# elucideye/acf

Hardware: AMD Instinct MI355X
Metric: detector FPS @1080p, 8 scales/octave, FACE80 model (higher is better)
Workload: dtype f32

## Files before the change

### acf_amd/csrc/kernels_levels.hip.h

```cpp
#pragma once

namespace acfhip
{

struct RsX
{
    int xa, m;
    float w[4];
    int wofs;
    bool border;
};

__device__ __forceinline__ float rs_C(int xmode, int ha, const RsX& X, const float* __restrict__ ft,
    const float* __restrict__ A, int row)
{
    if (row >= ha)
    {
        return 0.f;
    }
    const float* A0 = A + int64_t(X.xa) * ha + row;
    if (xmode == RS_EXACT)
    {
        float s = A0[0] + A0[ha];
        if (X.m > 2)
// ... 240 lines not shown
        const float a5 = Ac0[r4], b5 = Ac1[r4];
        float ar[5], br[5];
#pragma unroll
        for (int i = 0; i < 5; i++)
        {
            const int j = sh + i;
            ar[i] = j == 0 ? a4.x : (j == 1 ? a4.y : (j == 2 ? a4.z : (j == 3 ? a4.w : a5)));
            br[i] = j == 0 ? b4.x : (j == 1 ? b4.y : (j == 2 ? b4.z : (j == 3 ? b4.w : b5)));
        }
        float C[5];
#pragma unroll
        for (int i = 0; i < 5; i++)
        {
            const float c = border ? ar[i] : ar[i] * w0 + br[i] * w1;
            C[i] = live[i] ? c : 0.f;
        }
        float v[4];
#pragma unroll
        for (int k = 0; k < 4; k++)
        {
            const float c0 = i0[k] == 0 ? C[0] : (i0[k] == 1 ? C[1] : (i0[k] == 2 ? C[2] : C[3]));
            const float c1 = i0[k] == 0 ? C[1] : (i0[k] == 1 ? C[2] : (i0[k] == 2 ? C[3] : C[4]));
            const float o1 = c0 * wy0[k];
            v[k] = one[k] ? o1 : o1 + c1 * wy1[k];
        }
        if (act)
        {
            *reinterpret_cast<float4*>(B + int64_t(xb) * hb + yb0) = make_float4(v[0], v[1], v[2], v[3]);
        }
    }
}

struct RankFn
{
    int32_t shift, base, nbm1;
    uint32_t mask;
};
__device__ __forceinline__ uint4 rank_fetch(float v, const RankFn& f, const uint4* rec, uint32_t& low)
{
    const int key = __float_as_int(v);
    int b;
    asm("v_med3_i32 %0, %1, 0, %2" : "=v"(b) : "v"((key >> f.shift) - f.base), "v"(f.nbm1));
    low = (uint32_t(key) & f.mask) | 0x8000u;
    return rec[b];
}
__device__ __forceinline__ uint32_t rank_count(float v, const uint4& r, uint32_t low)
{
    static_assert(RANK_WINDOW == 7 && sizeof(RankRec) == 16 && RANK_UNUSED == 0x8000, "record layout");
    const uint32_t X = low | (low << 16);
    const uint32_t m0 = (X - r.x) & 0x00008000u;
    const uint32_t m1 = (X - r.y) & 0x80008000u;
    const uint32_t m2 = (X - r.z) & 0x80008000u;
    const uint32_t m3 = (X - r.w) & 0x80008000u;
    const uint32_t n = uint32_t(__builtin_popcount(m0 | (m1 >> 1) | (m2 >> 2) | (m3 >> 3))) + (r.x >> 16);
    return v < 0.f ? 0u : n;
}
__device__ __forceinline__ uint32_t rank_cell(float v, const RankFn& f, const uint4* rec)
{
    uint32_t low;
    const uint4 r = rank_fetch(v, f, rec, low);
    return rank_count(v, r, low);
}

__device__ __forceinline__ RankFn rank_tables_to_lds(const RankChan& rc, const RankRec* __restrict__ recG, uint4* recL, int tid, int nThreads)
{
    const uint4* src = reinterpret_cast<const uint4*>(recG + rc.recOff);
    for (int i = tid; i < rc.nb; i += nThreads)
    {
        recL[i] = src[i];
    }
    RankFn f;
    f.shift = rc.shift;
    f.base = rc.base;
    f.nbm1 = rc.nb - 1;
    f.mask = (1u << rc.shift) - 1u;
    return f;
}

struct RankJob
{
    int64_t src_off;
    int64_t dst_off;
    int32_t hP, wP, pitchR, pad_;
};
constexpr int RANK_CHUNK_COLS = 64;
__global__ void __launch_bounds__(256) k_rank(const float* __restrict__ pyr, int64_t pyr_fs, uint16_t* __restrict__ out, int64_t out_fs,
    const RankJob* __restrict__ jobs, int nChns, const RankChan* __restrict__ chan, const RankRec* __restrict__ recG)
{
    extern __shared__ uint4 ldsRec[];
    const int lvl = blockIdx.y / nChns, z = blockIdx.y - lvl * nChns;
    const RankJob J = jobs[lvl];
    const int c0 = blockIdx.x * RANK_CHUNK_COLS;
    if (c0 >= J.wP)
    {
        return;
    }
    const RankFn fn = rank_tables_to_lds(chan[z], recG, ldsRec, threadIdx.x, 256);
    __syncthreads();
    const float* __restrict__ src = pyr + int64_t(blockIdx.z) * pyr_fs + J.src_off + int64_t(z) * J.hP * J.wP;
    uint16_t* __restrict__ dst = out + int64_t(blockIdx.z) * out_fs + J.dst_off + int64_t(z) * J.pitchR * J.wP;
    const int c1 = min(c0 + RANK_CHUNK_COLS, J.wP);
    const int lane = threadIdx.x & 63, wv = threadIdx.x >> 6;
    for (int c = c0 + wv; c < c1; c += 4)
    {
        for (int r = lane; r < J.hP; r += 64)
        {
            dst[int64_t(c) * J.pitchR + r] = uint16_t(rank_cell(src[int64_t(c) * J.hP + r], fn, ldsRec));
        }
    }
}

struct LevelJob
{
    int32_t hC, wC, out_cs, desc;
    int32_t kind, pad_;
    int64_t in_off;
    int64_t raw_off;
    int64_t out_off;
    int64_t in_ps, out_ps;
    int64_t rank_off, rank_ps;
    int32_t rank_cs, pad2_;
};


typedef uint32_t u32x8 __attribute__((ext_vector_type(8)));
typedef const __attribute__((address_space(4))) u32x8* cptr8_t;

enum
{
    LM_REAL = 0,
    LM_DD = 1,
    LM_DU = 2,
    LM_UD = 3,
    LM_UU = 4
};

typedef __amdgpu_buffer_rsrc_t srd_t;
__device__ __forceinline__ srd_t make_srd(const void* base, int64_t bytes)
{
    const uint64_t a = reinterpret_cast<uint64_t>(base);
    const uint32_t lo = __builtin_amdgcn_readfirstlane(uint32_t(a)), hi = __builtin_amdgcn_readfirstlane(uint32_t(a >> 32));
    const uint32_t n = __builtin_amdgcn_readfirstlane(uint32_t(bytes > 0xffffffffll ? 0xffffffffll : bytes));
    void* p = reinterpret_cast<void*>((uint64_t(hi) << 32) | lo);
    return __builtin_amdgcn_make_buffer_rsrc(p, 0, int(n), 0x00020000);
}
__device__ __forceinline__ float buf_ld(srd_t r, uint32_t voff, uint32_t soff)
{
    return __uint_as_float(__builtin_amdgcn_raw_buffer_load_b32(r, voff, soff, 0));
}
__device__ __forceinline__ void buf_st(srd_t r, uint32_t voff, uint32_t soff, float v)
{
    __builtin_amdgcn_raw_buffer_store_b32(__float_as_uint(v), r, voff, soff, 0);
}

#ifndef ACF_LEVEL_WAVES
#define ACF_LEVEL_WAVES 4
#endif
constexpr int LEVEL_WAVES = ACF_LEVEL_WAVES;
constexpr int LEVEL_RING_FLOATS = 2304;
constexpr int LEVEL_RING_FLOATS_RANK = 1920;

template <int R, int MODE, int RING = LEVEL_RING_FLOATS>
struct LevelWindow
{
    static constexpr bool XDOWN = MODE == LM_DD || MODE == LM_DU;
    static constexpr bool YDOWN = MODE == LM_DD || MODE == LM_UD;
    static constexpr int NY = YDOWN ? 3 : 2;
    static constexpr int JX = XDOWN ? 3 : 2;
    static constexpr int RS = YDOWN ? (3 * R + 1) / 2 : R;
    static constexpr int NBRAW = RING / (RS * 64);
    static constexpr int NB = NBRAW > 12 ? 12 : (NBRAW < JX + 2 ? JX + 2 : NBRAW);
    static constexpr int LA = NB - JX;
    static constexpr int LDS_FLOATS = RS * 64 * (NB + 1);
    static_assert(LA * RS <= 63, "vmcnt immediate");

    uint32_t srow[RS];
    int issued;
    float* ring;

    __device__ __forceinline__ void request(srd_t A, int col, int ha, int wa) const
    {
        const uint32_t cb = uint32_t(min(col, wa - 1)) * uint32_t(ha) * 4u;
        float* slot = ring + (uint32_t(col) % uint32_t(NB)) * (RS * 64);
#pragma unroll
        for (int r = 0; r < RS; r++)
        {
            __builtin_amdgcn_raw_ptr_buffer_load_lds(A, (lptr_t)(slot + 64 * r), 4, srow[r], cb, 0, 0);
        }
    }

    __device__ __forceinline__ void init(srd_t A, float* ring_, int lane, int ha, int wa, int xa0)
    {
#pragma unroll
        for (int r = 0; r < RS; r++)
        {
            srow[r] = lane + 64 * r < ha ? 4u * uint32_t(lane + 64 * r) : 0x40000000u;
        }
        ring = ring_;
        for (int k = 0; k < JX + LA; k++)
        {
            request(A, xa0 + k, ha, wa);
        }
        issued = xa0 + JX + LA - 1;
    }

    __device__ __forceinline__ void advance(srd_t A, int xa, int ha, int wa)
    {
        const int target = xa + JX - 1 + LA;
        while (issued < target)
        {
            issued++;
            request(A, issued, ha, wa);
        }
    }

    __device__ __forceinline__ void read(float (&d)[JX][RS], int xa, int lane) const
    {
        asm volatile("s_waitcnt vmcnt(%0)" ::"n"(LA * RS) : "memory");
#pragma unroll
        for (int j = 0; j < JX; j++)
        {
            const float* slot = ring + (uint32_t(xa + j) % uint32_t(NB)) * (RS * 64) + lane;
#pragma unroll
            for (int r = 0; r < RS; r++)
            {
                d[j][r] = slot[64 * r];
            }
        }
    }
};

template <int R>
struct LaneTaps
{
    uint32_t roff[R][3];
    float wy[R][3];
    uint32_t one[R];
};

template <int R, int MODE, int RING>
__device__ __forceinline__ void level_column(float (&v)[R], int xb, srd_t A, int h, const uint32_t (&yoff)[R],
    int ha, int wa, int ny, const u32x8& xr, const LaneTaps<R>& tp, srd_t raw, bool haveRaw, bool lastOk,
    LevelWindow<R, MODE == LM_REAL ? LM_DD : MODE, RING>& win, float* ldsCol, int lane)
{
    if (MODE == LM_REAL)
    {
        const uint32_t col = uint32_t(xb) * uint32_t(h) * 4u;
#pragma unroll
        for (int k = 0; k < R; k++)
        {
            v[k] = buf_ld(A, yoff[k], col);
        }
        return;
    }
    constexpr bool XDOWN = MODE == LM_DD || MODE == LM_DU;
    constexpr bool YDOWN = MODE == LM_DD || MODE == LM_UD;
    typedef LevelWindow<R, MODE == LM_REAL ? LM_DD : MODE, RING> Win;
    constexpr int NY = Win::NY;
    constexpr int JX = Win::JX;
    const int xa = int(xr[0]), m = int(xr[1]);
    const bool border = xr[3] != 0;
    float w[4] = { __uint_as_float(xr[4]), __uint_as_float(xr[5]), __uint_as_float(xr[6]), __uint_as_float(xr[7]) };
    constexpr int RS = Win::RS;
    if (RS >= 3 && RS < 6)
    {
        ACF_PIN_V(w[0]);
        ACF_PIN_V(w[1]);
        ACF_PIN_V(w[2]);
    }
    win.advance(A, xa, ha, wa);
    float sc[JX][RS];
    win.read(sc, xa, lane);
    float Cr[RS];
    if (XDOWN)
    {
        if (m == 2)
        {
#pragma unroll
            for (int r = 0; r < RS; r++)
            {
                Cr[r] = sc[0][r] * w[0] + sc[1][r] * w[1];
            }
        }
        else if (m >= 3)
        {
#pragma unroll
            for (int r = 0; r < RS; r++)
            {
                Cr[r] = sc[0][r] * w[0] + sc[1][r] * w[1] + sc[JX - 1][r] * w[2];
            }
        }
        else
        {
#pragma unroll
            for (int r = 0; r < RS; r++)
            {
                Cr[r] = sc[0][r] * w[0];
            }
        }
    }
    else if (border)
    {
#pragma unroll
        for (int r = 0; r < RS; r++)
        {
            Cr[r] = sc[0][r];
        }
    }
    else
    {
#pragma unroll
        for (int r = 0; r < RS; r++)
        {
            Cr[r] = sc[0][r] * w[0] + sc[1][r] * w[1];
        }
    }
#pragma unroll
    for (int r = 0; r < RS; r++)
    {
        ldsCol[lane + 64 * r] = Cr[r];
    }
    float C[R][NY];
#pragma unroll
    for (int k = 0; k < R; k++)
    {
#pragma unroll
        for (int o = 0; o < NY; o++)
        {
            C[k][o] = *reinterpret_cast<const float*>(reinterpret_cast<const char*>(ldsCol) + tp.roff[k][o]);
        }
    }
    if (YDOWN)
    {
        if (ny > 2)
        {
#pragma unroll
            for (int k = 0; k < R; k++)
            {
                v[k] = C[k][0] * tp.wy[k][0] + C[k][1] * tp.wy[k][1] + C[k][2] * tp.wy[k][2];
            }
        }
        else
        {
#pragma unroll
            for (int k = 0; k < R; k++)
            {
                v[k] = C[k][0] * tp.wy[k][0] + C[k][1] * tp.wy[k][1];
            }
        }
    }
    else
    {
#pragma unroll
        for (int k = 0; k < R; k++)
        {
            const float o1 = C[k][0] * tp.wy[k][0];
            const float o2 = o1 + C[k][1] * tp.wy[k][1];
            v[k] = tp.one[k] ? o1 : o2;
        }
    }
    if (haveRaw)
    {
        const uint32_t rc = uint32_t(xb) * uint32_t(h) * 4u;
#pragma unroll
        for (int k = 0; k < R; k++)
        {
            if (k < R - 1 || lastOk)
            {
                buf_st(raw, yoff[k], rc, v[k]);
            }
        }
    }
}

enum
{
    LO_F32 = 1,
    LO_RANK = 2
};
struct LevelRank
{
    uint16_t* out;
    int64_t fs;
    RankFn fn;
    const uint4* rec;
};

struct LevelSeg
{
    int x0, x1, xs;
    float* spec;
    float* tru;
};

template <int R, int MODE, int OUT, int SEG>
__device__ __forceinline__ void level_body(const LevelJob& J, const int64_t f, const float* __restrict__ chns, float* __restrict__ pyr, float* __restrict__ rawOut,
    const ResampleDesc* __restrict__ descs, const int32_t* __restrict__ it, const float* __restrict__ ft,
    int nChns, int64_t chns_fs, int64_t pyr_fs, float p, float* __restrict__ dump, float* ldsBlock, int ldsWaveFloats, const LevelRank& rk,
    const LevelSeg& sg)
{
    const int z = __builtin_amdgcn_readfirstlane(blockIdx.x);
    const int lane = threadIdx.x & 63;
    const int h = J.hC, w = J.wC;
    const srd_t Osrd = make_srd(pyr + f * pyr_fs + J.out_off + int64_t(z) * J.out_ps, (int64_t(w - 1) * J.out_cs + h) * 4);
    const int par = int(J.rank_off & 1);
    const srd_t Rsrd = (OUT & LO_RANK) ? make_srd(rk.out + f * rk.fs + (J.rank_off - par) + int64_t(z) * J.rank_ps, (int64_t(w - 1) * J.rank_cs + h + 1 + par) * 2) : Osrd;
    srd_t A, raw = Osrd;
    bool haveRaw = false;
    int ha = 0, wa = 0, ny = 0;
    LaneTaps<R> tp;
    uint32_t yoff[R];
#pragma unroll
    for (int k = 0; k < R; k++)
    {
        yoff[k] = 4u * uint32_t(min(lane + 64 * k, h - 1));
    }
    const bool lastOk = lane + 64 * (R - 1) < h;
    const int32_t* xcol = it;
    if (MODE == LM_REAL)
    {
        A = make_srd(chns + f * chns_fs + J.in_off + int64_t(z) * J.in_ps, J.in_ps * 4);
    }
    else
    {
        const ResampleDesc& d = descs[J.desc];
        A = make_srd(chns + f * chns_fs + d.src_off + int64_t(z) * d.ha * d.wa, int64_t(d.ha) * d.wa * 4);
        haveRaw = rawOut != nullptr;
        if (haveRaw)
        {
            raw = make_srd(rawOut + f * chns_fs + J.raw_off + int64_t(z) * J.in_ps, J.in_ps * 4);
        }
        const int ty = z < d.c1 ? 0 : (z < d.c2 ? 1 : 2);
        const float r = d.r[ty];
        const int hb = d.hb;
        ha = d.ha;
        wa = d.wa;
        xcol = it + d.x_col;
        constexpr bool YDOWN = MODE == LM_DD || MODE == LM_UD;
        typedef LevelWindow<R, MODE == LM_REAL ? LM_DD : MODE> Win0;
        ny = YDOWN ? d.ybd0 : 2;
#pragma unroll
        for (int k = 0; k < R; k++)
        {
            const int ybc = int(yoff[k] >> 2);
            int ya;
            tp.wy[k][0] = tp.wy[k][1] = tp.wy[k][2] = 0.f;
            tp.one[k] = 0;
            if (YDOWN)
            {
                const int q0 = it[d.y_start + ybc];
                ya = it[d.y_src + q0];
#pragma unroll
                for (int o = 0; o < 3; o++)
                {
                    if (o < d.ybd0)
                    {
                        tp.wy[k][o] = ft[d.y_wt + q0 + o] * r;
                    }
                }
            }
            else
            {
                ya = it[d.y_src + ybc];
                tp.wy[k][0] = ft[d.y_wt + ybc] * r;
                tp.wy[k][1] = r - tp.wy[k][0];
                tp.one[k] = (ybc < d.ybd0 || ybc >= hb - d.ybd1) ? 1u : 0u;
            }
#pragma unroll
            for (int o = 0; o < 3; o++)
            {
                tp.roff[k][o] = 4u * uint32_t(min(ya + o, 64 * Win0::RS - 1));
            }
        }
    }
    float nrm = 1.0f / ((p + 2) * (p + 2));
    const float p1 = 1 + p;
    float pv = p;
    if (R <= 5)
    {
        ACF_PIN_V(nrm);
        ACF_PIN_V(pv);
    }
    cptr8_t xrec = (cptr8_t)(uintptr_t)xcol;
    const u32x8 zrec = { 0, 0, 0, 0, 0, 0, 0, 0 };
    float b0[R], b1[R], b2[R], b3[R], prev[R];
#pragma unroll
    for (int k = 0; k < R; k++)
    {
        b0[k] = b1[k] = b2[k] = b3[k] = prev[k] = 0.f;
    }
    const int xs = SEG ? sg.xs : 0, x0 = SEG ? sg.x0 : 0, x1 = SEG ? sg.x1 : w;
    u32x8 xr = (MODE == LM_REAL) ? zrec : xrec[xs];
    u32x8 xrn = (MODE == LM_REAL) ? zrec : xrec[min(xs + 1, w - 1)];
    constexpr int RING = (OUT & LO_RANK) ? LEVEL_RING_FLOATS_RANK : LEVEL_RING_FLOATS;
    typedef LevelWindow<R, MODE == LM_REAL ? LM_DD : MODE, RING> Win;
    Win lw;
    float* ldsCol = ldsBlock + (threadIdx.x >> 6) * ldsWaveFloats;
    if (MODE != LM_REAL)
    {
        lw.init(A, ldsCol + Win::RS * 64, lane, ha, wa, int(xr[0]));
    }
    const int lastLane = (h - 1) & 63;
#define LV_LOAD(FAR, COL)                                                                                           \
    {                                                                                                               \
        level_column<R, MODE, RING>(FAR, min((COL), w - 1), A, h, yoff, ha, wa, ny, xr, tp, raw, haveRaw, lastOk, lw, ldsCol, lane); \
        xr = xrn;                                                                                                   \
        xrn = (MODE == LM_REAL) ? zrec : xrec[min((COL) + 2, w - 1)];                                               \
    }
#define LV_FILTER(I, CUR, NXT)                                                                                      \
    {                                                                                                               \
        const int i_ = (I);                                                                                         \
        float T[R], up[R], dn[R];                                                                                   \
        _Pragma("unroll") for (int k = 0; k < R; k++)                                                               \
        {                                                                                                           \
            const float Im = CUR[k];                                                                                \
            const float Ir = (i_ < w - 1) ? NXT[k] : Im;                                                            \
            const float Il = (i_ == xs) ? Im : prev[k];  \
            T[k] = nrm * (Il + pv * Im + Ir);                                                                       \
            up[k] = wave_ror1(T[k]);                                                    \
            dn[k] = wave_rol1(T[k]);                                                    \
        }                                                                                                           \
        _Pragma("unroll") for (int k = 0; k < R; k++)                                                               \
        {                                                                                                           \
            const int y = lane + 64 * k;                                                                            \
            const float tm = (lane == 0) ? up[k > 0 ? k - 1 : 0] : up[k];                              \
            const float tpv = (lane == 63) ? dn[k + 1 < R ? k + 1 : k] : dn[k];                        \
            const float mid = tm + pv * T[k] + tpv;                                                                 \
             \
             \
            float o = mid;                                                                                          \
            if (k == R - 1)                                                                                         \
            {                                                                                                       \
                o = (y == h - 1) ? tm + p1 * T[k] : o;                                                              \
            }                                                                                                       \
            if (k == 0)                                                                                             \
            {                                                                                                       \
                o = (y == 0) ? p1 * T[k] + tpv : o;                                                                 \
            }                                                                                                       \
            prev[k] = o;                                                                                            \
             \
             \
            const float ov = (k < R - 1 || lastOk) ? o : __int_as_float(__builtin_amdgcn_readlane(__float_as_int(o), lastLane)); \
            if (OUT & LO_F32)                                                                                       \
            {                                                                                                       \
                   \
                buf_st(Osrd, yoff[k], (!SEG || i_ >= x0) ? uint32_t(i_) * uint32_t(J.out_cs) * 4u : 0x40000000u, ov); \
            }                                                                                                       \
        }                                                                                                           \
    }
    uint4 rrec[R];
    uint32_t rlow[R];
    uint32_t rvoff[R];
    if (OUT & LO_RANK)
    {
#pragma unroll
        for (int k = 0; k < R; k++)
        {
            const int y = lane + 64 * k;
            rvoff[k] = (((y + par) & 1) && y <= h) ? uint32_t(2 * (y - 1 + par)) : 0x40000000u;
        }
    }
#define LV_RANK_FETCH()                                                                                             \
    if (OUT & LO_RANK)                                                                                              \
    {                                                                                                               \
        _Pragma("unroll") for (int k = 0; k < R; k++)                                                               \
        {                                                                                                           \
            rrec[k] = rank_fetch(prev[k], rk.fn, rk.rec, rlow[k]);                                                  \
        }                                                                                                           \
    }
#define LV_RANK_STORE(COL)                                                                                          \
    if (OUT & LO_RANK)                                                                                              \
    {                                                                                                               \
        const int c_ = (COL);                                                                                       \
        const uint32_t so_ = c_ >= x0 ? uint32_t(c_) * uint32_t(J.rank_cs) * 2u : 0x40000000u;                      \
        uint32_t n_[R], up_[R];                                                                                     \
        _Pragma("unroll") for (int k = 0; k < R; k++)                                                               \
        {                                                                                                           \
            n_[k] = rank_count(prev[k], rrec[k], rlow[k]);                                                          \
            up_[k] = __float_as_uint(wave_ror1(__uint_as_float(n_[k])));        \
        }                                                                                                           \
        _Pragma("unroll") for (int k = 0; k < R; k++)                                                               \
        {                                                                                                           \
            const uint32_t lo_ = (lane == 0) ? up_[k > 0 ? k - 1 : 0] : up_[k];                                     \
            __builtin_amdgcn_raw_buffer_store_b32((n_[k] << 16) | (lo_ & 0xffffu), Rsrd, rvoff[k], so_, 0);         \
        }                                                                                                           \
    }
    LV_LOAD(b0, xs);
    LV_LOAD(b1, xs + 1);
    LV_LOAD(b2, xs + 2);
    const srd_t Ssrd = (SEG && sg.spec) ? make_srd(sg.spec, int64_t(h) * 4) : Osrd;
    int i = xs;
    for (; i + 3 < x1; i += 4)
    {
        if (SEG)
        {
            const uint32_t ss_ = (sg.spec && i == x0) ? 0u : 0x40000000u;
#pragma unroll
            for (int k = 0; k < R; k++)
            {
                buf_st(Ssrd, yoff[k], ss_, prev[k]);
            }
        }
        LV_RANK_FETCH();
        LV_LOAD(b3, i + 3);
        LV_RANK_STORE(i - 1);
        LV_FILTER(i, b0, b1);
        LV_RANK_FETCH();
        LV_LOAD(b0, i + 4);
        LV_RANK_STORE(i);
        LV_FILTER(i + 1, b1, b2);
        LV_RANK_FETCH();
        LV_LOAD(b1, i + 5);
        LV_RANK_STORE(i + 1);
        LV_FILTER(i + 2, b2, b3);
        LV_RANK_FETCH();
        LV_LOAD(b2, i + 6);
        LV_RANK_STORE(i + 2);
        LV_FILTER(i + 3, b3, b0);
    }
    if (SEG && sg.spec && i == x0)
    {
#pragma unroll
        for (int k = 0; k < R; k++)
        {
            buf_st(Ssrd, yoff[k], 0u, prev[k]);
        }
    }
    if (i < x1)
    {
        LV_RANK_FETCH();
        LV_RANK_STORE(i - 1);
        LV_FILTER(i, b0, b1);
    }
    if (i + 1 < x1)
    {
        LV_RANK_FETCH();
        LV_RANK_STORE(i);
        LV_FILTER(i + 1, b1, b2);
    }
    if (i + 2 < x1)
    {
        LV_RANK_FETCH();
        LV_RANK_STORE(i + 1);
        LV_FILTER(i + 2, b2, b2);
    }
    LV_RANK_FETCH();
    LV_RANK_STORE(x1 - 1);
    if (SEG && sg.tru)
    {
        const srd_t Tsrd = make_srd(sg.tru, int64_t(h) * 4);
#pragma unroll
        for (int k = 0; k < R; k++)
        {
            buf_st(Tsrd, yoff[k], 0u, prev[k]);
        }
    }
#undef LV_RANK_FETCH
#undef LV_RANK_STORE
#undef LV_LOAD
#undef LV_FILTER
}

template <int R, int MODE>
constexpr int levelWaveFloats()
{
    return MODE == LM_REAL ? 1 : LevelWindow<R, MODE == LM_REAL ? LM_DD : MODE>::LDS_FLOATS;
}
template <int R, int MODE>
__global__ void __launch_bounds__(64 * LEVEL_WAVES) __attribute__((amdgpu_waves_per_eu(R <= 4 ? 4 : 1))) k_level(const float* __restrict__ chns, float* __restrict__ pyr, float* __restrict__ rawOut,
    const LevelJob* __restrict__ jobs, const ResampleDesc* __restrict__ descs, const int32_t* __restrict__ it, const float* __restrict__ ft,
    int nChns, int64_t chns_fs, int64_t pyr_fs, float p, float* __restrict__ dump, int nFrames)
{
    const LevelJob J = jobs[blockIdx.y];
    constexpr int WF = levelWaveFloats<R, MODE>();
    __shared__ float ldsBlock[LEVEL_WAVES * WF];
    const int f = __builtin_amdgcn_readfirstlane(int(blockIdx.z) * LEVEL_WAVES + int(threadIdx.x >> 6));
    if (f >= nFrames)
    {
        return;
    }
    const LevelRank rk{};
    const LevelSeg sg{};
    level_body<R, MODE, LO_F32, 0>(J, f, chns, pyr, rawOut, descs, it, ft, nChns, chns_fs, pyr_fs, p, dump, ldsBlock, WF, rk, sg);
}

#define ACF_LEVEL_KIND(R, M) ((R) * 8 + (M))
constexpr int LEVEL_ALL_WF = LevelWindow<4, LM_DD>::LDS_FLOATS;
constexpr int LEVEL_ALL_WF_RANK = LevelWindow<4, LM_DD, LEVEL_RING_FLOATS_RANK>::LDS_FLOATS;
struct LevelRankArgs
{
    uint16_t* out;
    int64_t fs;
    const RankChan* chan;
    const RankRec* rec;
};
struct LevelSegArgs
{
    int32_t nSeg, warm, hMax, nJobs;
    float* spec;
    float* tru;
    int32_t* redo;
};
template <int OUT, int SEG>
__global__ void __launch_bounds__(64 * LEVEL_WAVES) __attribute__((amdgpu_waves_per_eu(4))) k_level_all(const float* __restrict__ chns, float* __restrict__ pyr, float* __restrict__ rawOut,
    const LevelJob* __restrict__ jobs, const ResampleDesc* __restrict__ descs, const int32_t* __restrict__ it, const float* __restrict__ ft,
    int nChns, int64_t chns_fs, int64_t pyr_fs, float p, float* __restrict__ dump, int nFrames, LevelRankArgs ra, LevelSegArgs sa)
{
    const int job = SEG ? int(blockIdx.z) / sa.nSeg : int(blockIdx.z);
    const LevelJob J = jobs[job];
    constexpr int RING = (OUT & LO_RANK) ? LEVEL_RING_FLOATS_RANK : LEVEL_RING_FLOATS;
    constexpr int WF = (OUT & LO_RANK) ? LEVEL_ALL_WF_RANK : LEVEL_ALL_WF;
    static_assert(LevelWindow<3, LM_DD, RING>::LDS_FLOATS <= WF && LevelWindow<4, LM_UU, RING>::LDS_FLOATS <= WF && LevelWindow<2, LM_DD, RING>::LDS_FLOATS <= WF &&
                      LevelWindow<3, LM_UU, RING>::LDS_FLOATS <= WF && LevelWindow<1, LM_DD, RING>::LDS_FLOATS <= WF,
        "ring size");
    extern __shared__ float ldsBlock[];
    LevelRank rk{};
    if ((OUT & LO_RANK) != 0)
    {
        uint4* recL = reinterpret_cast<uint4*>(ldsBlock + LEVEL_WAVES * WF);
        rk.fn = rank_tables_to_lds(ra.chan[blockIdx.x], ra.rec, recL, threadIdx.x, 64 * LEVEL_WAVES);
        rk.out = ra.out;
        rk.fs = ra.fs;
        rk.rec = recL;
        __syncthreads();
    }
    const int f = __builtin_amdgcn_readfirstlane(int(blockIdx.y) * LEVEL_WAVES + int(threadIdx.x >> 6));
    if (f >= nFrames)
    {
        return;
    }
    LevelSeg sg{};
    if (SEG)
    {
        const int64_t plane = (int64_t(f) * sa.nJobs + job) * nChns + blockIdx.x;
        if (sa.redo)
        {
            if (sa.redo[plane] == 0)
            {
                return;
            }
            if ((threadIdx.x & 63) == 0)
            {
                sa.redo[plane] = 0;
            }
        }
        const int seg = int(blockIdx.z) - job * sa.nSeg;
        const int nSegJ = max(1, min(sa.nSeg, J.wC / (2 * sa.warm)));
        if (seg >= nSegJ)
        {
            return;
        }
        const int segW = ((J.wC + nSegJ - 1) / nSegJ + 3) & ~3;
        sg.x0 = seg * segW;
        sg.x1 = min(sg.x0 + segW, J.wC);
        sg.xs = max(sg.x0 - sa.warm, 0);
        if (sg.x0 >= sg.x1)
        {
            return;
        }
        const bool lastSeg = sg.x1 >= J.wC;
        sg.spec = seg > 0 ? sa.spec + (plane * sa.nSeg + seg) * int64_t(sa.hMax) : nullptr;
        sg.tru = !lastSeg ? sa.tru + (plane * sa.nSeg + seg + 1) * int64_t(sa.hMax) : nullptr;
    }
#define LV_CASE(RR, MM)                                                                                                       \
    case ACF_LEVEL_KIND(RR, MM):                                                                                               \
        level_body<RR, MM, OUT, SEG>(J, f, chns, pyr, rawOut, descs, it, ft, nChns, chns_fs, pyr_fs, p, dump, ldsBlock, WF, rk, sg); \
        break;
#define LV_CASES(RR) LV_CASE(RR, LM_REAL) LV_CASE(RR, LM_DD) LV_CASE(RR, LM_UU)
    switch (J.kind)
    {
        LV_CASES(1)
        LV_CASES(2)
        LV_CASES(3)
        LV_CASES(4)
        LV_CASE(5, LM_REAL)
        LV_CASE(6, LM_REAL)
        LV_CASE(7, LM_REAL)
        LV_CASE(8, LM_REAL)
        default:
            break;
    }
#undef LV_CASES
#undef LV_CASE
}

__global__ void __launch_bounds__(64) k_level_verify(const float* __restrict__ spec, const float* __restrict__ tru, const LevelJob* __restrict__ jobs,
    LevelSegArgs sa, int nChns, int32_t* __restrict__ redo, int force)
{
    const int job = int(blockIdx.x) / sa.nSeg, seg = int(blockIdx.x) - job * sa.nSeg;
    const LevelJob J = jobs[job];
    const int nSegJ = max(1, min(sa.nSeg, J.wC / (2 * sa.warm)));
    const int segW = ((J.wC + nSegJ - 1) / nSegJ + 3) & ~3;
    if (seg == 0 || seg >= nSegJ || seg * segW >= J.wC)
    {
        return;
    }
    const int64_t plane = (int64_t(blockIdx.z) * sa.nJobs + job) * nChns + blockIdx.y;
    const uint32_t* a = reinterpret_cast<const uint32_t*>(spec) + (plane * sa.nSeg + seg) * int64_t(sa.hMax);
    const uint32_t* b = reinterpret_cast<const uint32_t*>(tru) + (plane * sa.nSeg + seg) * int64_t(sa.hMax);
    bool bad = force != 0;
    for (int y = threadIdx.x; y < J.hC; y += 64)
    {
        bad = bad || (a[y] != b[y]);
    }
    if (bad)
    {
        redo[plane] = 1;
    }
// ... 30 lines not shown
```

### acf_amd/csrc/plan_build.hip.h

```cpp
#pragma once

namespace
{
struct PlanBuild
{
    acf_hip_ctx* const c;
    const acf_hip_params& p;
    Plan& pl;
    const int H, W, d_in, B, max_hits, shrink, d;
    const int64_t np0;
    TableArena arena;
    std::vector<SmoothJob> realJobs, finalJobList;
    std::vector<int64_t> rankOffs;
    std::vector<PadJob> padJobs, padJobsR;
    int py = 0, px = 0;

    PlanBuild(acf_hip_ctx* ctx, int H_, int W_, int d_in_, int max_batch, int max_hits_)
        : c(ctx), p(ctx->p), pl(ctx->plan), H(H_), W(W_), d_in(d_in_), B(max_batch), max_hits(max_hits_), shrink(ctx->p.shrink), d(ctx->plan.d), np0(int64_t(H_) * W_)
    {
    }
    int colourBuffer();
    int realScales();
    int imageStrips();
    int approxLevels();
// ... 178 lines not shown
    c->nApproxDescs = int(c->h_descs.size()) - c->nImgDescs;
    c->autoLambdas = p.nApprox > 0 && p.nLambdas != 3;
    c->h_lambdas.assign(size_t(B) * 3, 0.0);
    if (c->autoLambdas && (rc = devAlloc(c, &c->d_planeSums, size_t(B) * 2 * pl.nChns)))
    {
        return rc;
    }

    return ACF_HIP_OK;
}

int PlanBuild::finalJobs()
{
    int rc = ACF_HIP_OK;
    (void)rc;
    int64_t rankOff = 0;
    c->finalMaxH = 0;
    c->padMaxElems = 0;
    py = p.pad_h / shrink;
    px = p.pad_w / shrink;
    for (size_t i = 0; i < pl.levels.size(); i++)
    {
        const acf_hip_level& l = pl.levels[i];
        SmoothJob j{};
        j.h = l.hC;
        j.w = l.wC;
        j.nplanes = pl.nChns;
        j.out_cs = l.hP;
        j.in_off = pl.raw_off[i];
        j.out_off = l.offset + int64_t(px) * l.hP + py;
        j.in_ps = int64_t(l.hC) * l.wC;
        j.out_ps = int64_t(l.hP) * l.wP;
        finalJobList.push_back(j);
        c->finalMaxH = std::max(c->finalMaxH, l.hC);
        PadJob q{};
        q.hC = l.hC;
        q.wC = l.wC;
        q.hP = l.hP;
        q.wP = l.wP;
        q.py = py;
        q.px = px;
        q.nplanes = pl.nChns;
        q.pitch = l.hP;
        q.off = l.offset;
        padJobs.push_back(q);
        q.pitch = rankPitch(l.hP);
        q.off = rankOff;
        padJobsR.push_back(q);
        c->padMaxElems = std::max<int64_t>(c->padMaxElems, int64_t(pl.nChns) * (int64_t(l.wP) * (l.hP - l.hC) + int64_t(l.wP - l.wC) * l.hC));
        rankOffs.push_back(rankOff);
        rankOff += int64_t(pl.nChns) * rankPitch(l.hP) * l.wP;
    }
    return ACF_HIP_OK;
}

int PlanBuild::levelJobs()
{
    int rc = ACF_HIP_OK;
    (void)rc;
    {
        struct Keyed
        {
            int key;
            LevelJob j;
        };
        std::vector<Keyed> fusedJobs, rawJobs;
        c->fusedOk = p.smooth > 0 && c->finalMaxH <= 64 * LEVEL_MAX_R_REAL;
        int ai = 0;
        for (size_t i = 0; i < pl.levels.size(); i++)
        {
            const acf_hip_level& l = pl.levels[i];
            LevelJob j{};
            j.hC = l.hC;
            j.wC = l.wC;
            j.out_cs = l.hP;
            j.in_off = pl.raw_off[i];
            j.raw_off = pl.raw_off[i];
            j.out_off = l.offset + int64_t(px) * l.hP + py;
            j.in_ps = int64_t(l.hC) * l.wC;
            j.out_ps = int64_t(l.hP) * l.wP;
            j.rank_cs = rankPitch(l.hP);
            j.rank_ps = int64_t(j.rank_cs) * l.wP;
            j.rank_off = rankOffs[i] + int64_t(px) * j.rank_cs + py;
            j.desc = -1;
            const int R = (l.hC + 63) / 64;
            int mode = LM_REAL;
            rawJobs.push_back({ R * 8 + LM_REAL, j });
            if (!l.isReal)
            {
                j.desc = ai;
                const ResampleDesc& dd = c->h_descs[size_t(c->nImgDescs + ai)];
                if ((dd.ymode == RS_DOWN && dd.ybd0 > 3) || (dd.xmode == RS_DOWN && dd.xbd0 > 3) || dd.ymode == RS_EXACT || dd.xmode == RS_EXACT)
                {
                    c->fusedOk = false;
                }
                mode = dd.xmode == RS_DOWN ? (dd.ymode == RS_DOWN ? LM_DD : LM_DU) : (dd.ymode == RS_DOWN ? LM_UD : LM_UU);
                if (R > 8)
                {
                    c->fusedOk = false;
                }
                if (dd.ha >= 64 * (dd.ymode == RS_DOWN ? (3 * R + 1) / 2 : R))
                {
                    c->fusedOk = false;
                }
                if (mode == LM_DU || mode == LM_UD)
                {
                    c->fusedOk = false;
                }
                ai++;
            }
            fusedJobs.push_back({ R * 8 + mode, j });
        }
        auto pack = [&](std::vector<Keyed>& v, std::vector<acf_hip_ctx::LevelGroup>& groups, LevelJob** dst, int* nAll) {
            auto jobCost = [](const Keyed& k) {
                const int R = k.key / 8, mode = k.key % 8;
                return double(k.j.wC) * (R * (mode == LM_REAL ? 1.0 : 3.0) + 2.0);
            };
            for (auto& k : v)
            {
                k.j.kind = k.key;
            }
            std::vector<Keyed> all, rest;
            for (const auto& k : v)
            {
                const int R = k.key / 8, mode = k.key % 8;
                ((R <= 4 || (mode == LM_REAL && R <= 8)) && !fallbackForced(FB_LEVEL_GROUPS) ? all : rest).push_back(k);
            }
            std::stable_sort(all.begin(), all.end(), [&](const Keyed& a, const Keyed& b) { return jobCost(a) > jobCost(b); });
            std::stable_sort(rest.begin(), rest.end(), [](const Keyed& a, const Keyed& b) { return a.key < b.key; });
            std::vector<LevelJob> flat;
            for (const auto& k : all)
            {
                flat.push_back(k.j);
            }
            *nAll = int(all.size());
            groups.clear();
            for (const auto& k : rest)
            {
                if (groups.empty() || groups.back().R * 8 + groups.back().mode != k.key)
                {
                    groups.push_back({ k.key / 8, k.key % 8, int(flat.size()), 0, 0.0, 0 });
                }
                groups.back().count++;
                groups.back().cost += jobCost(k);
                flat.push_back(k.j);
            }
            return devUpload(c, dst, flat);
        };
        if ((rc = pack(fusedJobs, c->levelGroups, &c->d_levelJobs, &c->nAllJobs)) || (rc = pack(rawJobs, c->levelGroupsRaw, &c->d_levelJobsRaw, &c->nAllJobsRaw)))
        {
            return rc;
        }
        c->levelsEmitRank = c->fusedOk && c->levelGroups.empty() && c->nAllJobs == int(pl.levels.size());
        for (const auto& l : pl.levels)
        {
            if ((py & 1) && l.hC % 64 == 0)
            {
                c->levelsEmitRank = false;
            }
        }
    }
    return ACF_HIP_OK;
}

int PlanBuild::ldcf()
{
    int rc = ACF_HIP_OK;
    LdcfStage& L = c->ldcf;
    if (p.ldcfK <= 0)
    {
        return ACF_HIP_OK;
    }
    const int shrink2 = 2 * p.shrink, nCk = pl.nChns * p.ldcfK;
    L.descBase = int(c->h_descs.size());
    L.tmpFloats = int64_t(p.ldcfK) * pl.pyr_floats;
    std::vector<LdcfJob> jobs;
    for (size_t i = 0; i < pl.levels.size(); i++)
    {
        acf_hip_level l = pl.levels[i];
        const acf_hip_level& s0 = pl.levels[i];
        l.hP = l.hC = int(std::floor(0.5 * s0.hP + 0.5));
        l.wP = l.wC = int(std::floor(0.5 * s0.wP + 0.5));
        if (l.hP < 1 || l.wP < 1)
        {
            return fail(c, ACF_HIP_E_UNSUPPORTED, "plan: LDCF level smaller than one cell");
        }
        l.nWinR = std::max(0, int(std::ceil(float(l.hP * shrink2 - p.modelDsPad_h + 1) / p.stride)));
        l.nWinC = std::max(0, int(std::ceil(float(l.wP * shrink2 - p.modelDsPad_w + 1) / p.stride)));
        l.offset = L.floats;
        L.floats += int64_t(nCk) * l.hP * l.wP;
        L.levels.push_back(l);
        ResampleDesc dd;
        if ((rc = buildResample(s0.hP, s0.wP, l.hP, l.wP, dd, arena)))
        {
            return fail(c, rc, "plan: degenerate LDCF resample geometry");
        }
        const double one[3] = { 1.0, 1.0, 1.0 };
        setResampleGain(dd, one, nCk, nCk);
        dd.nplanes = nCk;
        dd.src_off = int64_t(p.ldcfK) * s0.offset;
        dd.dst_off = l.offset;
        dd.src_frame_stride = L.tmpFloats;
        c->h_descs.push_back(dd);
        LdcfJob j{};
        j.h = s0.hP;
        j.w = s0.wP;
        j.inOff = s0.offset;
        j.outOff = int64_t(p.ldcfK) * s0.offset;
        jobs.push_back(j);
        L.maxCells = std::max(L.maxCells, s0.hP * s0.wP);
        L.maxBlocks = std::max(L.maxBlocks, resampleBlocks(dd));
    }
    for (size_t i = 0; i < L.levels.size(); i++)
    {
        c->h_descs[size_t(L.descBase) + i].dst_frame_stride = L.floats;
    }
    std::vector<LdcfTileJob> tj;
    bool ok = !fallbackForced(FB_LDCF_UNFUSED);
    const int xoMax = 16;
    std::vector<std::pair<int, int>> cand;
    for (int y = RT_YO; y >= 32; y--)
    {
        for (int x = xoMax; x >= xoMax / 2; x--)
        {
            cand.push_back({ y, x });
        }
    }
    std::stable_sort(cand.begin(), cand.end(), [](const std::pair<int, int>& a, const std::pair<int, int>& b) { return a.first * a.second > b.first * b.second; });
    for (size_t i = 0; i < L.levels.size() && ok; i++)
    {
        const ResampleDesc& dd = c->h_descs[size_t(L.descBase) + i];
        ResampleTiling tl;
        int yo = 0, xo = 0;
        for (const auto& yx : cand)
        {
            tl = resampleTilePlan(dd, arena, yx.second, int64_t(40) * 1024, yx.first, 128, 2 * xoMax);
            if (tl.rows > 0)
            {
                yo = yx.first;
                xo = yx.second;
                break;
            }
        }
        if (tl.rows <= 0)
        {
            ok = false;
            break;
        }
        L.tileRows = std::max(L.tileRows, tl.rows);
        L.tileCols = std::max(L.tileCols, tl.cols);
        const int ntY = cdiv(dd.hb, yo), ntX = cdiv(dd.wb, xo);
        for (int x = 0; x < ntX; x++)
        {
            for (int y = 0; y < ntY; y++)
            {
                LdcfTileJob j{};
                j.level = int(i);
                j.ytile = y;
                j.xtile = x;
                j.tile_y = tl.tile_y;
                j.tile_x = tl.tile_x;
                j.yo = yo;
                j.xo = xo;
                tj.push_back(j);
            }
        }
    }
    if (ok && !tj.empty())
    {
        L.tiles = int(tj.size());
        if ((rc = devUpload(c, &L.d_tileJobs, tj)))
        {
            return rc;
        }
    }
    if ((rc = devUpload(c, &L.d_jobs, jobs)) || (rc = devUpload(c, &L.d_filt, L.filters)) ||
        (L.tiles == 0 && (rc = devAlloc(c, &L.d_tmp, size_t(B) * L.tmpFloats + 64))) || (rc = devAlloc(c, &L.d_pyr, size_t(B) * L.floats + 64)))
    {
        return rc;
    }
    return ACF_HIP_OK;
}

int PlanBuild::uploadAndScratch()
{
    int rc = ACF_HIP_OK;
    (void)rc;
    if ((rc = devUpload(c, &c->d_descs, c->h_descs)) || (rc = devUpload(c, &c->d_it, arena.ints)) || (rc = devUpload(c, &c->d_ft, arena.floats)) ||
        (rc = devUpload(c, &c->d_realJobs, realJobs)) || (rc = devUpload(c, &c->d_finalJobs, finalJobList)) || (rc = devUpload(c, &c->d_padJobs, padJobs)) || (rc = devUpload(c, &c->d_padJobsR, padJobsR)))
    {
        return rc;
    }
    if ((rc = devAlloc(c, &c->d_chns, size_t(B) * pl.raw_floats)) || (rc = devAlloc(c, &c->d_pyr, size_t(B) * pl.pyr_floats + 64)) )
    {
        return rc;
    }
    {
        c->segCap = 32;
        const size_t nState = size_t(B) * d * c->segCap * size_t(std::max(H, 4));
        if ((rc = devAlloc(c, &c->d_specState, nState)) || (rc = devAlloc(c, &c->d_trueState, nState)) || (rc = devAlloc(c, &c->d_redo, size_t(B) * d)))
        {
            return rc;
        }
        HIPCHK(c, hipMemsetAsync(c->d_redo, 0, sizeof(int32_t) * size_t(B) * d, c->stream));
        HIPCHK(c, hipStreamSynchronize(c->stream));
        c->redoInts = size_t(B) * d;
    }
    {
        c->levelSegFrames = std::min(B, 8);
        c->levelSegCap = 8;
        c->levelHMax = std::max(c->finalMaxH, 4);
        const size_t nState = size_t(c->levelSegFrames) * pl.levels.size() * pl.nChns * c->levelSegCap * size_t(c->levelHMax);
        if ((rc = devAlloc(c, &c->d_lvSpec, nState)) || (rc = devAlloc(c, &c->d_lvTrue, nState)) ||
// ... 33 lines not shown
```

Baseline: 16550.

## Give each lane contiguous rows so level loads and stores become vector buffer ops

```diff
diff --git a/acf_amd/csrc/kernels_levels.hip.h b/acf_amd/csrc/kernels_levels.hip.h
--- a/acf_amd/csrc/kernels_levels.hip.h
+++ b/acf_amd/csrc/kernels_levels.hip.h
@@ -416,6 +416,61 @@
 {
     __builtin_amdgcn_raw_buffer_store_b32(__float_as_uint(v), r, voff, soff, 0);
 }
+typedef uint32_t u32x2 __attribute__((ext_vector_type(2)));
+typedef uint32_t u32x3 __attribute__((ext_vector_type(3)));
+typedef uint32_t u32x4 __attribute__((ext_vector_type(4)));
+template <int R, int K = 0>
+__device__ __forceinline__ void buf_ld_rows(float (&v)[R], srd_t r, uint32_t voff, uint32_t soff)
+{
+    constexpr int N = R - K;
+    if constexpr (N >= 4)
+    {
+        const u32x4 t = __builtin_amdgcn_raw_buffer_load_b128(r, voff + 4u * K, soff, 0);
+        v[K] = __uint_as_float(t.x), v[K + 1] = __uint_as_float(t.y), v[K + 2] = __uint_as_float(t.z), v[K + 3] = __uint_as_float(t.w);
+        buf_ld_rows<R, K + 4>(v, r, voff, soff);
+    }
+    else if constexpr (N == 3)
+    {
+        const u32x3 t = __builtin_amdgcn_raw_buffer_load_b96(r, voff + 4u * K, soff, 0);
+        v[K] = __uint_as_float(t.x), v[K + 1] = __uint_as_float(t.y), v[K + 2] = __uint_as_float(t.z);
+    }
+    else if constexpr (N == 2)
+    {
+        const u32x2 t = __builtin_amdgcn_raw_buffer_load_b64(r, voff + 4u * K, soff, 0);
+        v[K] = __uint_as_float(t.x), v[K + 1] = __uint_as_float(t.y);
+    }
+    else if constexpr (N == 1)
+    {
+        v[K] = buf_ld(r, voff + 4u * K, soff);
+    }
+}
+__device__ __forceinline__ uint32_t dword_of(float v) { return __float_as_uint(v); }
+__device__ __forceinline__ uint32_t dword_of(uint32_t v) { return v; }
+template <int R, int K = 0, typename T>
+__device__ __forceinline__ void buf_st_rows(srd_t r, uint32_t voff, uint32_t soff, const T (&v)[R])
+{
+    constexpr int N = R - K;
+    if constexpr (N >= 4)
+    {
+        const u32x4 t = { dword_of(v[K]), dword_of(v[K + 1]), dword_of(v[K + 2]), dword_of(v[K + 3]) };
+        __builtin_amdgcn_raw_buffer_store_b128(t, r, voff + 4u * K, soff, 0);
+        buf_st_rows<R, K + 4>(r, voff, soff, v);
+    }
+    else if constexpr (N == 3)
+    {
+        const u32x3 t = { dword_of(v[K]), dword_of(v[K + 1]), dword_of(v[K + 2]) };
+        __builtin_amdgcn_raw_buffer_store_b96(t, r, voff + 4u * K, soff, 0);
+    }
+    else if constexpr (N == 2)
+    {
+        const u32x2 t = { dword_of(v[K]), dword_of(v[K + 1]) };
+        __builtin_amdgcn_raw_buffer_store_b64(t, r, voff + 4u * K, soff, 0);
+    }
+    else if constexpr (N == 1)
+    {
+        __builtin_amdgcn_raw_buffer_store_b32(dword_of(v[K]), r, voff + 4u * K, soff, 0);
+    }
+}
 
 #ifndef ACF_LEVEL_WAVES
 #define ACF_LEVEL_WAVES 4
@@ -503,18 +558,14 @@
 };
 
 template <int R, int MODE, int RING>
-__device__ __forceinline__ void level_column(float (&v)[R], int xb, srd_t A, int h, const uint32_t (&yoff)[R],
-    int ha, int wa, int ny, const u32x8& xr, const LaneTaps<R>& tp, srd_t raw, bool haveRaw, bool lastOk,
+__device__ __forceinline__ void level_column(float (&v)[R], int xb, srd_t A, int h, uint32_t yld, uint32_t yst,
+    int ha, int wa, int ny, const u32x8& xr, const LaneTaps<R>& tp, srd_t raw, bool haveRaw,
     LevelWindow<R, MODE == LM_REAL ? LM_DD : MODE, RING>& win, float* ldsCol, int lane)
 {
     if (MODE == LM_REAL)
     {
         const uint32_t col = uint32_t(xb) * uint32_t(h) * 4u;
-#pragma unroll
-        for (int k = 0; k < R; k++)
-        {
-            v[k] = buf_ld(A, yoff[k], col);
-        }
+        buf_ld_rows<R>(v, A, yld, col);
         return;
     }
     constexpr bool XDOWN = MODE == LM_DD || MODE == LM_DU;
@@ -625,15 +676,7 @@
     }
     if (haveRaw)
     {
-        const uint32_t rc = uint32_t(xb) * uint32_t(h) * 4u;
-#pragma unroll
-        for (int k = 0; k < R; k++)
-        {
-            if (k < R - 1 || lastOk)
-            {
-                buf_st(raw, yoff[k], rc, v[k]);
-            }
-        }
+        buf_st_rows<R>(raw, yst, uint32_t(xb) * uint32_t(h) * 4u, v);
     }
 }
 
@@ -673,13 +716,12 @@
     bool haveRaw = false;
     int ha = 0, wa = 0, ny = 0;
     LaneTaps<R> tp;
-    uint32_t yoff[R];
-#pragma unroll
-    for (int k = 0; k < R; k++)
-    {
-        yoff[k] = 4u * uint32_t(min(lane + 64 * k, h - 1));
-    }
-    const bool lastOk = lane + 64 * (R - 1) < h;
+    const int nl = (h + R - 1) / R, nShort = nl * R - h;
+    const bool shortL = R > 1 && lane < nShort;
+    const bool active = lane < nl;
+    const int row0 = min(shortL ? lane * (R - 1) : lane * R - nShort, h - R);
+    const uint32_t yld = 4u * uint32_t(row0);
+    const uint32_t yst = active ? yld : 0x40000000u;
     const int32_t* xcol = it;
     if (MODE == LM_REAL)
     {
@@ -706,7 +748,7 @@
 #pragma unroll
         for (int k = 0; k < R; k++)
         {
-            const int ybc = int(yoff[k] >> 2);
+            const int ybc = row0 + k;
             int ya;
             tp.wy[k][0] = tp.wy[k][1] = tp.wy[k][2] = 0.f;
             tp.one[k] = 0;
@@ -764,64 +806,68 @@
     {
         lw.init(A, ldsCol + Win::RS * 64, lane, ha, wa, int(xr[0]));
     }
-    const int lastLane = (h - 1) & 63;
 #define LV_LOAD(FAR, COL)                                                                                           \
     {                                                                                                               \
-        level_column<R, MODE, RING>(FAR, min((COL), w - 1), A, h, yoff, ha, wa, ny, xr, tp, raw, haveRaw, lastOk, lw, ldsCol, lane); \
+        level_column<R, MODE, RING>(FAR, min((COL), w - 1), A, h, yld, yst, ha, wa, ny, xr, tp, raw, haveRaw, lw, ldsCol, lane); \
         xr = xrn;                                                                                                   \
         xrn = (MODE == LM_REAL) ? zrec : xrec[min((COL) + 2, w - 1)];                                               \
     }
 #define LV_FILTER(I, CUR, NXT)                                                                                      \
     {                                                                                                               \
         const int i_ = (I);                                                                                         \
-        float T[R], up[R], dn[R];                                                                                   \
+        float T[R], o_[R];                                                                                          \
         _Pragma("unroll") for (int k = 0; k < R; k++)                                                               \
         {                                                                                                           \
             const float Im = CUR[k];                                                                                \
             const float Ir = (i_ < w - 1) ? NXT[k] : Im;                                                            \
             const float Il = (i_ == xs) ? Im : prev[k];  \
             T[k] = nrm * (Il + pv * Im + Ir);                                                                       \
-            up[k] = wave_ror1(T[k]);                                                    \
-            dn[k] = wave_rol1(T[k]);                                                    \
         }                                                                                                           \
+         \
+         \
+        const float up = wave_ror1(shortL ? T[R > 1 ? R - 2 : 0] : T[R - 1]);                                       \
+        const float dn0 = wave_rol1(T[0]);                                                                          \
+        const float dn = shortL ? wave_rol1(T[R > 1 ? 1 : 0]) : dn0;                                                \
         _Pragma("unroll") for (int k = 0; k < R; k++)                                                               \
         {                                                                                                           \
-            const int y = lane + 64 * k;                                                                            \
-            const float tm = (lane == 0) ? up[k > 0 ? k - 1 : 0] : up[k];                              \
-            const float tpv = (lane == 63) ? dn[k + 1 < R ? k + 1 : k] : dn[k];                        \
+            const float tm = k > 0 ? T[k > 0 ? k - 1 : 0] : up;                                        \
+            const float tpv = k + 1 < R ? T[k + 1 < R ? k + 1 : k] : dn;                               \
             const float mid = tm + pv * T[k] + tpv;                                                                 \
              \
              \
             float o = mid;                                                                                          \
             if (k == R - 1)                                                                                         \
             {                                                                                                       \
-                o = (y == h - 1) ? tm + p1 * T[k] : o;                                                              \
+                o = (lane == nl - 1) ? tm + p1 * T[k] : o;                                                          \
             }                                                                                                       \
             if (k == 0)                                                                                             \
             {                                                                                                       \
-                o = (y == 0) ? p1 * T[k] + tpv : o;                                                                 \
+                o = (lane == 0) ? p1 * T[k] + tpv : o;                                                              \
             }                                                                                                       \
-            prev[k] = o;                                                                                            \
-             \
-             \
-            const float ov = (k < R - 1 || lastOk) ? o : __int_as_float(__builtin_amdgcn_readlane(__float_as_int(o), lastLane)); \
-            if (OUT & LO_F32)                                                                                       \
-            {                                                                                                       \
+            prev[k] = o_[k] = o;                                                                                    \
+        }                                                                                                           \
+        if (OUT & LO_F32)                                                                                           \
+        {                                                                                                           \
                    \
-                buf_st(Osrd, yoff[k], (!SEG || i_ >= x0) ? uint32_t(i_) * uint32_t(J.out_cs) * 4u : 0x40000000u, ov); \
-            }                                                                                                       \
+            buf_st_rows<R>(Osrd, yst, (!SEG || i_ >= x0) ? uint32_t(i_) * uint32_t(J.out_cs) * 4u : 0x40000000u, o_); \
         }                                                                                                           \
     }
     uint4 rrec[R];
     uint32_t rlow[R];
-    uint32_t rvoff[R];
+    uint32_t rvoff = 0x40000000u, rvlast = 0x40000000u, rsh = 0;
     if (OUT & LO_RANK)
     {
-#pragma unroll
-        for (int k = 0; k < R; k++)
-        {
-            const int y = lane + 64 * k;
-            rvoff[k] = (((y + par) & 1) && y <= h) ? uint32_t(2 * (y - 1 + par)) : 0x40000000u;
+        const int c0 = row0 + par;
+        const bool odd = (c0 & 1) != 0;
+        rsh = odd ? 0u : 16u;
+        rvoff = active ? uint32_t(2 * (c0 & ~1)) : 0x40000000u;
+        if (R & 1)
+        {
+            rvlast = (active && (odd || lane == nl - 1)) ? rvoff + 4u * uint32_t(R / 2) : 0x40000000u;
+        }
+        else
+        {
+            rvlast = (odd && lane == nl - 1) ? uint32_t(2 * (c0 + R - 1)) : 0x40000000u;
         }
     }
 #define LV_RANK_FETCH()                                                                                             \
@@ -837,17 +883,27 @@
     {                                                                                                               \
         const int c_ = (COL);                                                                                       \
         const uint32_t so_ = c_ >= x0 ? uint32_t(c_) * uint32_t(J.rank_cs) * 2u : 0x40000000u;                      \
-        uint32_t n_[R], up_[R];                                                                                     \
+        uint32_t n_[R], V_[R / 2 + 1];                                                                              \
         _Pragma("unroll") for (int k = 0; k < R; k++)                                                               \
         {                                                                                                           \
             n_[k] = rank_count(prev[k], rrec[k], rlow[k]);                                                          \
-            up_[k] = __float_as_uint(wave_ror1(__uint_as_float(n_[k])));        \
         }                                                                                                           \
-        _Pragma("unroll") for (int k = 0; k < R; k++)                                                               \
+        const uint32_t nUp_ = __float_as_uint(wave_ror1(__uint_as_float(shortL ? n_[R > 1 ? R - 2 : 0] : n_[R - 1]))); \
+        _Pragma("unroll") for (int q = 0; q <= R / 2; q++)                                                          \
         {                                                                                                           \
-            const uint32_t lo_ = (lane == 0) ? up_[k > 0 ? k - 1 : 0] : up_[k];                                     \
-            __builtin_amdgcn_raw_buffer_store_b32((n_[k] << 16) | (lo_ & 0xffffu), Rsrd, rvoff[k], so_, 0);         \
+            const uint32_t lo_ = q > 0 ? n_[q > 0 ? 2 * q - 1 : 0] : nUp_;                                          \
+            V_[q] = ((2 * q < R ? n_[2 * q < R ? 2 * q : 0] : 0u) << 16) | (lo_ & 0xffffu);                         \
         }                                                                                                           \
+        if (R >= 2)                                                                                                 \
+        {                                                                                                           \
+            uint32_t D_[R >= 2 ? R / 2 : 1];                                                                        \
+            _Pragma("unroll") for (int q = 0; q < R / 2; q++)                                                       \
+            {                                                                                                       \
+                D_[q] = __builtin_amdgcn_alignbit(V_[q + 1], V_[q], rsh);                                           \
+            }                                                                                                       \
+            buf_st_rows<(R >= 2 ? R / 2 : 1)>(Rsrd, rvoff, so_, D_);                                                \
+        }                                                                                                           \
+        __builtin_amdgcn_raw_buffer_store_b32((R & 1) ? __builtin_amdgcn_alignbit(V_[R / 2], V_[R / 2], rsh) : V_[R / 2], Rsrd, rvlast, so_, 0); \
     }
     LV_LOAD(b0, xs);
     LV_LOAD(b1, xs + 1);
@@ -859,11 +915,7 @@
         if (SEG)
         {
             const uint32_t ss_ = (sg.spec && i == x0) ? 0u : 0x40000000u;
-#pragma unroll
-            for (int k = 0; k < R; k++)
-            {
-                buf_st(Ssrd, yoff[k], ss_, prev[k]);
-            }
+            buf_st_rows<R>(Ssrd, yst, ss_, prev);
         }
         LV_RANK_FETCH();
         LV_LOAD(b3, i + 3);
@@ -884,11 +936,7 @@
     }
     if (SEG && sg.spec && i == x0)
     {
-#pragma unroll
-        for (int k = 0; k < R; k++)
-        {
-            buf_st(Ssrd, yoff[k], 0u, prev[k]);
-        }
+        buf_st_rows<R>(Ssrd, yst, 0u, prev);
     }
     if (i < x1)
     {
@@ -913,11 +961,7 @@
     if (SEG && sg.tru)
     {
         const srd_t Tsrd = make_srd(sg.tru, int64_t(h) * 4);
-#pragma unroll
-        for (int k = 0; k < R; k++)
-        {
-            buf_st(Tsrd, yoff[k], 0u, prev[k]);
-        }
+        buf_st_rows<R>(Tsrd, yst, 0u, prev);
     }
 #undef LV_RANK_FETCH
 #undef LV_RANK_STORE
diff --git a/acf_amd/csrc/plan_build.hip.h b/acf_amd/csrc/plan_build.hip.h
--- a/acf_amd/csrc/plan_build.hip.h
+++ b/acf_amd/csrc/plan_build.hip.h
@@ -354,13 +354,6 @@
             return rc;
         }
         c->levelsEmitRank = c->fusedOk && c->levelGroups.empty() && c->nAllJobs == int(pl.levels.size());
-        for (const auto& l : pl.levels)
-        {
-            if ((py & 1) && l.hC % 64 == 0)
-            {
-                c->levelsEmitRank = false;
-            }
-        }
     }
     return ACF_HIP_OK;
 }
```

Result: no change. 16690 (median of 6 runs) (+0.9%).
